# aehogan/lammps-induced-dipole-polarization-pair-style

Hardware: AMD Instinct MI355X
Metric: atom-steps/sec (higher is better)
Workload: dtype f64

## Files before the change

lammps-induced-dipole-polarization-pair-style_amd/csrc/polar_api.hip:

```cpp
#include "polar_handle.hpp"

namespace {
void upload_types(polar_handle *h, int ntypes, const double *const t[7]) {
  need_device(h);
  std::vector<double> pack;
  const double r_cmax = pack_lj_table(ntypes, t, pack);
  h->d_lj.ensure(pack.size());
  HIPCHECK(hipMemcpy(h->d_lj.p, pack.data(), pack.size() * sizeof(double), hipMemcpyHostToDevice));
  h->P.ntypes = ntypes;
  h->P.ljpack = h->d_lj.p;
  h->ntypes = ntypes;
  h->types_set = true;
  h->r_cmax = r_cmax;
  h->skin_valid = false;
}

void upload_coul(polar_handle *h, double g_ewald, double qqrd2e, const double *slj, const double *scoul, int nbits,
                 int mask, int shift, double tabinnersq, const double *const t[8]) {
  need_device(h);
  h->P.g_ewald = g_ewald; h->P.qqrd2e = qqrd2e;
  for (int k = 0; k < 4; k++) { h->P.special_lj[k] = slj[k]; h->P.special_coul[k] = scoul[k]; }
  h->P.ncoultablebits = nbits; h->P.ncoulmask = mask; h->P.ncoulshiftbits = shift; h->P.tabinnersq = tabinnersq;
  std::vector<double> pack;
  pack_coul_table(nbits, t, pack);
// ... 156 lines not shown
    return POLAR_OK;
  }
  return guarded(h, [&]() {
    HIPCHECK(hipSetDevice(device));
    h->device_set = true;
    h->stream.create();
    for (auto &e : h->ev) e.create();
    {
      int prio_lo = 0, prio_hi = 0;
      HIPCHECK(hipDeviceGetStreamPriorityRange(&prio_lo, &prio_hi));
      h->lj_stream.create(hipStreamNonBlocking, prio_lo);
    }
    h->ev_fork.create(); h->ev_join.create();
    h->ev_lj0.create(); h->ev_lj1.create();
    h->ev_dl0.create(hipEventDisableTiming); h->ev_dl1.create(hipEventDisableTiming);
    h->ev_mu_ready.create(hipEventDisableTiming);
    for (auto &e : h->ev_fchunk) e.create(hipEventDisableTiming);
    for (auto &e : h->ev_ks) e.create();
    h->dl_stream.create(hipStreamNonBlocking);
    if (getenv("POLAR_NO_OVERLAP")) h->overlap_lj = false;
    if (const char *e = getenv("POLAR_LJ_PERS")) h->lj_pers = atoi(e);
    if (const char *e = getenv("POLAR_LJ_SKIN")) h->lj_skin = atoi(e) != 0;
    if (const char *e = getenv("POLAR_NL_INERT")) h->nl_inert = atoi(e) != 0;
    if (const char *e = getenv("POLAR_LJ_PERS_THREADS")) h->lj_pers_threads = std::max(256, std::min(POLAR_LJ_PERS_THREADS, (atoi(e) / 64) * 64));
    { int ncu = 0; if (hipDeviceGetAttribute(&ncu, hipDeviceAttributeMultiprocessorCount, device) == hipSuccess) h->ncu = ncu; }
    h->h_scal.ensure(1);
    h->h_flags.ensure(16);
    h->h_ddtot.ensure(64 * 16);
    h->d_overflow.ensure(16); h->d_ddtot.ensure(64 * 16);
    h->d_scal.ensure(1);
    h->d_slots.ensure((size_t)POLAR_NSLOT * POLAR_SLOT_STRIDE);
    h->have_device = true;
    return POLAR_OK;
  });
}

int polar_destroy(polar_handle *h) {
  if (!h) return POLAR_OK;
  delete h;
  return POLAR_OK;
}

const char *polar_last_error(const polar_handle *h) { return h ? h->err.c_str() : "null handle"; }
const char *polar_last_warning(const polar_handle *h) { return h ? h->warn.c_str() : ""; }

int polar_pair_settings(polar_handle *h, int narg, const char *const *arg) {
// ... 711 lines not shown
```

lammps-induced-dipole-polarization-pair-style_amd/csrc/polar_common.hpp:

```cpp
#pragma once

#include <hip/hip_runtime.h>
#include <stdint.h>

#ifdef POLAR_LAB
#define POLAR_LAB_PARAM , int ablate
#define POLAR_LAB_PASS , ablate
#define POLAR_ABL(bit) (ablate & (bit))
#else
#define POLAR_LAB_PARAM
#define POLAR_LAB_PASS
#define POLAR_ABL(bit) 0
#endif

namespace polar {


struct __attribute__((aligned(64))) AtomRec {
  double x, mx;
  double y, my;
  double z, mz;
  double q, a;
};

// ... 222 lines not shown

struct RecQuad { double2 a, b, c, d; };
__device__ __forceinline__ RecQuad fetch_records(const AtomRec *__restrict__ rec, int j, double2 *stage, int lane) {
  const int q4 = lane >> 2;
  const char *base = reinterpret_cast<const char *>(rec);
  const unsigned piece = (unsigned)(lane & 3) * 16u, k = lane & 3;
  const unsigned j0 = __shfl(j, q4, 64), j1 = __shfl(j, 16 + q4, 64), j2 = __shfl(j, 32 + q4, 64), j3 = __shfl(j, 48 + q4, 64);
  const double2 p0 = *reinterpret_cast<const double2 *>(base + ((j0 << 6) + piece));
  const double2 p1 = *reinterpret_cast<const double2 *>(base + ((j1 << 6) + piece));
  const double2 p2 = *reinterpret_cast<const double2 *>(base + ((j2 << 6) + piece));
  const double2 p3 = *reinterpret_cast<const double2 *>(base + ((j3 << 6) + piece));
  stage[q4 * 5 + k] = p0; stage[(16 + q4) * 5 + k] = p1;
  stage[(32 + q4) * 5 + k] = p2; stage[(48 + q4) * 5 + k] = p3;
  __builtin_amdgcn_fence(__ATOMIC_RELEASE, "wavefront");
  __builtin_amdgcn_wave_barrier();
  __builtin_amdgcn_fence(__ATOMIC_ACQUIRE, "wavefront");
  RecQuad r;
  r.a = stage[lane * 5]; r.b = stage[lane * 5 + 1]; r.c = stage[lane * 5 + 2]; r.d = stage[lane * 5 + 3];
  __builtin_amdgcn_wave_barrier();
  return r;
}

struct XQ { double2 a, b; };
__device__ __forceinline__ XQ fetch_xq(const double4 *__restrict__ xq, int j, double2 *stage, int lane) {
  const int h2 = lane >> 1;
  const char *base = reinterpret_cast<const char *>(xq);
  const unsigned piece = (unsigned)(lane & 1) * 16u, k = lane & 1;
  const unsigned j0 = __shfl(j, h2, 64), j1 = __shfl(j, 32 + h2, 64);
  const double2 p0 = *reinterpret_cast<const double2 *>(base + ((j0 << 5) + piece));
  const double2 p1 = *reinterpret_cast<const double2 *>(base + ((j1 << 5) + piece));
  stage[h2 * 3 + k] = p0; stage[(32 + h2) * 3 + k] = p1;
  __builtin_amdgcn_fence(__ATOMIC_RELEASE, "wavefront");
  __builtin_amdgcn_wave_barrier();
  __builtin_amdgcn_fence(__ATOMIC_ACQUIRE, "wavefront");
  XQ r;
  r.a = stage[lane * 3]; r.b = stage[lane * 3 + 1];
  __builtin_amdgcn_wave_barrier();
  return r;
}

struct ExpCoef {
  double log2e, ln2hi, ln2lo;
  double c[14];
};
inline ExpCoef make_expcoef() {
  ExpCoef K;
  K.log2e = 1.4426950408889634074; K.ln2hi = 6.93147180369123816490e-01; K.ln2lo = 1.90821492927058770002e-10;
  const double c[14] = {1.0, 1.0, 0.5, 0.16666666666666666, 0.041666666666666664, 0.008333333333333333, 0.001388888888888889, 0.0001984126984126984, 2.48015873015873e-05, 2.7557319223985893e-06, 2.755731922398589e-07, 2.505210838544172e-08, 2.08767569878681e-09, 1.6059043836821613e-10};
  for (int k = 0; k < 14; k++) K.c[k] = c[k];
  return K;
}
__device__ __forceinline__ double exp_neg(double x, const ExpCoef &K) {
  x = fmax(x, -745.0);
  const double n = rint(x * K.log2e);
  double r = fma(-n, K.ln2hi, x);
  r = fma(-n, K.ln2lo, r);
  double p = K.c[13];
#pragma unroll
  for (int k = 12; k >= 0; k--) p = fma(p, r, K.c[k]);
  return ldexp(p, (int)n);
}
// ... 88 lines not shown
```

lammps-induced-dipole-polarization-pair-style_amd/csrc/polar_handle.hpp:

```cpp
#pragma once
#include <hip/hip_runtime.h>

#include <algorithm>
#include <initializer_list>
#include <utility>
#include <chrono>
#include <cmath>
#include <cstdio>
#include <cstdlib>
#include <exception>
#include <cstring>
#include <numeric>
#include <string>
#include <thread>
#include <mutex>
#include <condition_variable>
#include <functional>
#include <memory>
#include <stdexcept>
#include <unistd.h>
#include <vector>

#include "pair_host.hpp"
#include "polar_input.hpp"
// ... 60 lines not shown
  DBuf<double> d_ef_s, d_T6, d_Minv, d_gsN, d_gsAT, d_cb, d_gs_part, d_eatom, d_vatom, d_dd_r2, d_fpol;
  bool dense_gs = false;
  CellGrid grid{};
  long long ncell = 0;
  bool sorted = false;
  DBuf<long long> d_first, d_sym_first;
  DBuf<int> d_gs_cnt;
  DBuf<long long> d_scan_a, d_scan_b;
  DBuf<int> d_sym_cnt, d_sym_fill, d_sym_j;
  bool sym_valid = false;
  DBuf<long long> d_sym_cfirst;
  DBuf<int> d_sym_cend, d_lj_walk;
  DBuf<unsigned char> d_sym_cls;
  DBuf<double4> d_xq_snap;
  DBuf<unsigned long long> d_lj_drift;
  double r_cmax = 0.0;
  int lj_skin = 1;
  bool skin_valid = false;
  int skin_nall = 0;
  bool lj_ran = false;
  bool lj_sym_last = false, lj_walk_last = false; int lj_rows_last = 0;
  double lj_walked = 0.0, lj_entries = 0.0;
  int nl_inert = 1;
  bool force_ran = false, force_listed = false; int force_nrows = 0;
  double nl_entries = 0.0, force_rows = 0.0;
  DBuf<unsigned long long> d_inert_sums;
  DBuf<AtomRec> d_rec0, d_rec1;
  DBuf<Scal> d_scal;
  DBuf<double> d_slots;
  DBuf<int> d_cell_id, d_cell_cnt, d_cell_fill, d_nl_cnt, d_dd_cnt, d_nl_j, d_dd_j, d_dd_wrap;
  DBuf<long long> d_cell_first, d_nl_first, d_dd_first;
  DBuf<double2> d_dd_s;
  DBuf<int2> d_lpdesc;
  DBuf<double> d_lp_pend;
  DBuf<double> d_lp_part;
  int lp_npart = 0;
  DBuf<int> d_slot;
  std::vector<int> h_cl;
  DBuf<int> d_cl_orig, d_cl_cnt, d_cl_wrap, d_cl_tw;
  DBuf<int4> d_cl_s;
  long long cl_pitch = 0;
  int ncl = 0;
  double cluster_dist = 2.0;
  int cluster_max = 4;
  long long cl_slots = 0;
  DBuf<double4> d_xq, d_pos4, d_xq_s;
  long long nl_pairs = 0, dd_pairs = 0;
  long long nl_pitch = 0, dd_pitch = 0;
  DBuf<int> d_overflow;
  DBuf<unsigned long long> d_ddtot;
  PinBuf<int> h_flags;
  PinBuf<unsigned long long> h_ddtot;
  int inum = 0;
// ... 301 lines not shown
```

lammps-induced-dipole-polarization-pair-style_amd/csrc/polar_lists.hpp:

```cpp
#pragma once

#include "polar_common.hpp"
#include "polar_nl_dense.hpp"

namespace polar {

struct CellGrid {
  int trim;
  int nc[3];
  double lo[3], inv[3];
};

__device__ __forceinline__ int cell_of(const CellGrid &g, const Box &b, double x, double y, double z) {
  int c[3];
  double fr3[3];
  frac_coords(b, g.lo, x, y, z, fr3);
#pragma unroll
  for (int k = 0; k < 3; k++) {
    double fr = fr3[k];
    fr -= floor(fr);
    int ck = (int)(fr * g.nc[k]);
    c[k] = ck >= g.nc[k] ? g.nc[k] - 1 : ck;
  }
  return (c[2] * g.nc[1] + c[1]) * g.nc[0] + c[0];
// ... 446 lines not shown

__device__ __forceinline__ int prefix_count(unsigned long long m, int base) {
  return __builtin_amdgcn_mbcnt_hi((unsigned)(m >> 32), __builtin_amdgcn_mbcnt_lo((unsigned)m, base));
}
struct NlRunLanes {
  int s0v, k0v, s1v, k1v, endv;
  unsigned m1;
  __device__ __forceinline__ int s0(int sr) const { return __builtin_amdgcn_readlane(s0v, sr); }
  __device__ __forceinline__ int k0(int sr) const { return __builtin_amdgcn_readlane(k0v, sr); }
  __device__ __forceinline__ int s1(int sr) const { return __builtin_amdgcn_readlane(s1v, sr); }
  __device__ __forceinline__ int k1(int sr) const { return __builtin_amdgcn_readlane(k1v, sr); }
  __device__ __forceinline__ int end(int sr) const { return __builtin_amdgcn_readlane(endv, sr); }
  __device__ __forceinline__ bool two(int sr) const { return (m1 >> sr) & 1u; }
};
template <bool TRI, bool RECHECK, bool DENSE = true>
static __global__ __launch_bounds__(POLAR_BLOCK) void k_nl_build(const int *__restrict__ rows, int nrows,
                                                          const double4 *__restrict__ pos4, Box box, CellGrid g,
                                                          const long long *__restrict__ cell_first, double cutallsq,
                                                          double ddcutsq, long long nl_pitch, long long dd_pitch,
                                                          int *__restrict__ nl_cnt, int *__restrict__ dd_cnt,
                                                          int *__restrict__ nl_j, int *__restrict__ dd_j,
                                                          double *__restrict__ dd_r2, int pad_dd,
                                                          int dd_shift_qm, int dd_pad_index, int *__restrict__ dd_wrap,
                                                          const int *__restrict__ color_s, double colordistsq,
                                                          int *__restrict__ color_conflict,
                                                          const int *__restrict__ dd_slot,
                                                          int *__restrict__ overflow,
                                                          unsigned long long *__restrict__ dd_total) {
  const int dd_shift = dd_shift_qm & 255, dd_qm = dd_shift_qm >> 8;
  const int lane = threadIdx.x & 63;
  const int row = blockIdx.x * POLAR_ROWS_PER_BLOCK + (threadIdx.x >> 6);
  if (row >= nrows) return;
  const int i = __builtin_amdgcn_readfirstlane(rows ? rows[row] : row);
  const double4 ri = pos4[i];
  const int imol = __double2hiint(ri.w), ipol = __double2loint(ri.w) >= SITE_POLAR;
  const int icol = (RECHECK && color_s && ipol) ? color_s[i] : -2;
  bool clash = RECHECK && color_s && ipol && icol < 0;
  int cc[3];
  double uu[3], edge[3];
  {
    double fr3[3];
    frac_coords(box, g.lo, ri.x, ri.y, ri.z, fr3);
#pragma unroll
    for (int k = 0; k < 3; k++) {
      double fr = fr3[k];
      fr -= floor(fr);
      const double t = fr * g.nc[k];
      int ck = (int)t;
      ck = ck >= g.nc[k] ? g.nc[k] - 1 : ck;
      cc[k] = __builtin_amdgcn_readfirstlane(ck);
      uu[k] = wave_uniform(t - ck); edge[k] = wave_uniform(box.prd[k] / g.nc[k]);
    }
  }
  const int c0 = cc[0], c1 = cc[1], c2 = cc[2];
  const int slot_i = __builtin_amdgcn_readfirstlane(dd_slot ? dd_slot[i] : i);
  const long long nl0 = (long long)i * nl_pitch, dd0 = (long long)(slot_i >= 0 ? slot_i : 0) * dd_pitch;
  char *const nl_row = reinterpret_cast<char *>(nl_j + nl0), *const dd_row = reinterpret_cast<char *>(dd_j + dd0);
  char *const r2_row = reinterpret_cast<char *>(dd_r2 ? dd_r2 + dd0 : nullptr);
  const char *const pos_b = reinterpret_cast<const char *>(pos4);
  const int nl_cap = (int)nl_pitch, dd_cap = (int)dd_pitch;
  const unsigned long long dd_im = (ipol && slot_i >= 0) ? ~0ull : 0ull;
  Box pbox = box;
#pragma unroll
  for (int k = 0; k < 3; k++) { pbox.inv[k] = box.periodic[k] ? box.inv[k] : 0.0; pbox.periodic[k] = 1; }
  int ncount = 0, dcount = 0;
  unsigned long long wrap_m = 0ull;
  const int same_i = imol != 0 ? POLAR_NL_SAMEMOL : 0;
  const unsigned long long below = (lane == 0) ? 0ull : (~0ull >> (64 - lane));
  const int n0 = g.nc[0], n1 = g.nc[1], n2 = g.nc[2];
  const int zlo = n2 >= 5 ? c2 - 2 : 0, zcnt = n2 >= 5 ? 5 : n2;
  const int ylo = n1 >= 5 ? c1 - 2 : 0, ycnt = n1 >= 5 ? 5 : n1;
  const double reach = sqrt(cutallsq > ddcutsq ? cutallsq : ddcutsq) + 1e-6;
  const double reach2 = wave_uniform(reach * reach);
  const int nsr = zcnt * ycnt;
  int ra0 = 0, rb0 = 0, ra1 = 0, rb1 = 0;
  if (lane < nsr) {
    const int lz = (lane >= ycnt) + (lane >= 2 * ycnt) + (lane >= 3 * ycnt) + (lane >= 4 * ycnt);
    const int zz = zlo + lz, yy = ylo + (lane - lz * ycnt);
    int b2 = zz, b1 = yy;
    bool ok = true;
    if (b2 < 0 || b2 >= n2) { if (!box.periodic[2]) ok = false; b2 = b2 < 0 ? b2 + n2 : b2 - n2; }
    if (b1 < 0 || b1 >= n1) { if (!box.periodic[1]) ok = false; b1 = b1 < 0 ? b1 + n1 : b1 - n1; }
    double dzmin = 0.0, dymin = 0.0;
    if (n2 >= 5) { const int d = zz - c2; dzmin = d > 0 ? (d - uu[2]) * edge[2] : (d < 0 ? (uu[2] - (d + 1)) * edge[2] : 0.0); }
    if (n1 >= 5) { const int d = yy - c1; dymin = d > 0 ? (d - uu[1]) * edge[1] : (d < 0 ? (uu[1] - (d + 1)) * edge[1] : 0.0); }
    const double rem2 = reach2 - dzmin * dzmin - dymin * dymin;
    if (g.trim && rem2 < 0.0) ok = false;
    int xlo = n0 >= 5 ? c0 - 2 : 0, xhi = n0 >= 5 ? c0 + 2 : n0 - 1;
    if (ok && g.trim && n0 >= 5) {
// ... 3 lines not shown
      xlo = c0 + lo_off; xhi = c0 + hi_off;
    }
    if (ok) {
      const long long rowbase = ((long long)b2 * n1 + b1) * n0;
      const int xa = xlo < 0 ? 0 : xlo, xb = xhi >= n0 ? n0 - 1 : xhi;
      ra0 = (int)cell_first[rowbase + xa]; rb0 = (int)cell_first[rowbase + xb + 1];
      if (box.periodic[0]) {
        if (xlo < 0) { ra1 = (int)cell_first[rowbase + xlo + n0]; rb1 = (int)cell_first[rowbase + n0]; }
        else if (xhi >= n0) { ra1 = (int)cell_first[rowbase]; rb1 = (int)cell_first[rowbase + xhi - n0 + 1]; }
      }
    }
  }
  auto candidate = [&](const int p, const bool valid) {
    const int j = valid ? p : i;
    const double4 rj = *reinterpret_cast<const double4 *>(pos_b + ((unsigned)j << 5));
    double ex, ey, ez;
    const unsigned long long shifted = min_image_rint_m<TRI>(pbox, ri.x, ri.y, ri.z, rj.x, rj.y, rj.z, ex, ey, ez);
    const double rsq = ex * ex + ey * ey + ez * ez;
    const unsigned long long m_pair = __builtin_amdgcn_ballot_w64(j != i);
    const int jkind = __double2loint(rj.w);
    const unsigned long long m_nl = m_pair & __builtin_amdgcn_ballot_w64(rsq <= cutallsq) & __builtin_amdgcn_ballot_w64(jkind != SITE_INERT);
    const unsigned long long m_dd = m_pair & dd_im & __builtin_amdgcn_ballot_w64(jkind >= SITE_POLAR) & __builtin_amdgcn_ballot_w64(rsq < ddcutsq);
    wrap_m |= m_dd & shifted;
    const bool in_nl = (j != i) & (rsq <= cutallsq) & (jkind != SITE_INERT);
    const bool in_dd = (j != i) & (dd_im != 0ull) & (jkind >= SITE_POLAR) & (rsq < ddcutsq);
    if (RECHECK) { if (icol >= 0 && j != i && rsq < colordistsq && jkind >= SITE_POLAR && color_s[j] == icol) clash = true; }
    int jmol = __double2hiint(rj.w);
    asm("" : "+v"(jmol));
    const int same = imol == jmol ? same_i : 0;
    const int kn = prefix_count(m_nl, ncount), kd = prefix_count(m_dd, dcount);
    if (in_nl && kn < nl_cap) *reinterpret_cast<int *>(nl_row + ((unsigned)kn << 2)) = j | same;
    if (in_dd && kd < dd_cap) {
      *reinterpret_cast<int *>(dd_row + ((dd_shift ? lp_slot32((unsigned)kd, dd_qm) : (unsigned)kd) << 2)) = j << dd_shift;
      if (dd_r2) *reinterpret_cast<double *>(r2_row + ((unsigned)kd << 3)) = rsq;
    }
    ncount += __popcll(m_nl);
    dcount += __popcll(m_dd);
  };
  if (DENSE) {
    const int len = nl_run_len(ra0, rb0, ra1, rb1);
    int inc = len;
    inc += __builtin_amdgcn_update_dpp(0, inc, 0x111, 0xF, 0xF, true);
    inc += __builtin_amdgcn_update_dpp(0, inc, 0x112, 0xF, 0xF, true);
    inc += __builtin_amdgcn_update_dpp(0, inc, 0x114, 0xF, 0xF, true);
    inc += __builtin_amdgcn_update_dpp(0, inc, 0x118, 0xF, 0xF, true);
    const int row0 = __builtin_amdgcn_readlane(inc, 15);
// ... 8 lines not shown
      candidate(g + k, g < total);
    }
  } else {
    for (int sr = 0; sr < nsr; sr++) {
#pragma unroll
      for (int piece = 0; piece < 2; piece++) {
        const int a = __builtin_amdgcn_readlane(piece ? ra1 : ra0, sr), b = __builtin_amdgcn_readlane(piece ? rb1 : rb0, sr);
        for (int base = a; base < b; base += 64) candidate(base + lane, base + lane < b);
      }
    }
  }
  if (pad_dd) {
    const int have = dcount < dd_pitch ? dcount : (int)dd_pitch;
    const int padded = (have + 63) & ~63;
    for (int k = have + lane; k < padded; k += 64) {
      dd_j[dd0 + (dd_shift ? lp_slot(k, dd_qm) : (long long)k)] = (dd_pad_index >= 0 ? dd_pad_index : i) << dd_shift;
      if (dd_r2) dd_r2[dd0 + k] = 1e60;
    }
  }
  if (RECHECK && color_s && __ballot(clash) != 0ull && lane == 0) atomicOr(color_conflict, 1);
  if (lane == 0) {
    nl_cnt[i] = ncount; dd_cnt[i] = dcount;
    if (dd_wrap) dd_wrap[i] = wrap_m != 0ull;
    if (ncount > nl_pitch || dcount > dd_pitch) atomicMax(overflow, ncount > dcount ? ncount : dcount);
    if (dcount) atomicAdd(dd_total + (blockIdx.x & 63) * 16, (unsigned long long)(dcount < dd_pitch ? dcount : (int)dd_pitch));
  }
}

#ifdef POLAR_LAB
#include "lab/lists_paired_rows.hpp"
#endif

#ifdef POLAR_LAB
#include "lab/lists_cluster_rows.hpp"
#endif

struct LJGrid {
  int nc[3];
  double lo[3], inv[3];
};
__device__ __forceinline__ int lj_cell_of(const LJGrid &g, double x, double y, double z) {
  const double p[3] = {x, y, z};
  int c[3];
#pragma unroll
  for (int k = 0; k < 3; k++) {
    int ck = (int)floor((p[k] - g.lo[k]) * g.inv[k]);
// ... 230 lines not shown
```

lammps-induced-dipole-polarization-pair-style_amd/csrc/polar_rows.hpp:

```cpp
#pragma once

#include "polar_common.hpp"
#include "polar_force_pair.hpp"
#include "polar_skin.hpp"
#ifdef POLAR_LAB
#include "lab/force_pair_literal.hpp"
#define POLAR_LIT_PARAM , int literal
#define POLAR_LIT_PASS , literal
#else
#define POLAR_LIT_PARAM
#define POLAR_LIT_PASS
#endif

namespace polar {

static __global__ void k_pack(int n, const int *__restrict__ perm, const double *__restrict__ x, const double *__restrict__ q,
                       const double *__restrict__ alpha, const int *__restrict__ mol, const double *__restrict__ mu0,
                       AtomRec *__restrict__ r0, AtomRec *__restrict__ r1, int *__restrict__ mol_s,
                       double4 *__restrict__ pos4, double4 *__restrict__ xq_s, int wrap, Box box, double lo0, double lo1,
                       double lo2, int keep_inert) {
  int i = blockIdx.x * blockDim.x + threadIdx.x;
  if (i == n) {
    AtomRec d;
    d.x = n > 0 ? x[0] : 0.0; d.y = n > 0 ? x[1] : 0.0; d.z = n > 0 ? x[2] : 0.0;
// ... 444 lines not shown
    const double2 fdf = bin[1], ede = bin[2];
    ctab_lds[b] = make_double4(fdf.x, fdf.y, ede.x, ede.y);
  }
  __syncthreads();
  const int lane = threadIdx.x & 63, wv = threadIdx.x >> 6, nwv = blockDim.x >> 6;
  double ev = 0.0, ec = 0.0;
  for (int ii = blockIdx.x + gridDim.x * wv; ii < inum; ii += gridDim.x * nwv) {
    const int i = ilist ? ilist[ii] : ii;
    const int jnum = numneigh ? numneigh[i] : (int)(first[i + 1] - first[i]);
    if (jnum == 0) continue;
    double v[6] = {0, 0, 0, 0, 0, 0};
    ljcoul_row<EFLAG, VPAIR, TAB>(P, i, jnum, neigh + first[i], xq[i], xq, type, lj_lds, ctab_lds, lane, f, eatom, vatom, ev, ec, v);
    if (VPAIR) ljcoul_tally<false, true>(slots, ii, lane, vglobal, 0.0, 0.0, v);
  }
  const double none[6] = {0, 0, 0, 0, 0, 0};
  ljcoul_tally<EFLAG, false>(slots, blockIdx.x * nwv + wv, lane, 0, ev, ec, none);
}

template <bool ALLPAIRS, bool EW>
static __device__ __forceinline__ void static_field_body(const int *__restrict__ rows, int nrows, int nlocal,
                                                              const AtomRec *__restrict__ rec,
                                                              const int *__restrict__ mol, Box box,
                                                              RowList nl,
                                                              const int *__restrict__ nl_j, double cut_coulsq,
                                                              double e2s, double gamma, int use_previous,
                                                              double *__restrict__ ef, AtomRec *__restrict__ rec0,
                                                              AtomRec *__restrict__ rec1, const double4 *__restrict__ xq_s,
                                                              double g_ewald, const double *__restrict__ erec) {
  const int lane = threadIdx.x & 63;
  const int row = blockIdx.x * POLAR_ROWS_PER_BLOCK + (threadIdx.x >> 6);
  if (row >= nrows) return;
  const int i = rows ? rows[row] : row;
  const AtomRec ri = uniform_rec(rec[i]);
  const int mi = mol[i];
  const double f_shift = -1.0 / cut_coulsq;
  double ex = 0, ey = 0, ez = 0;
  long long beg = 0, end = nlocal;
  if (!ALLPAIRS) row_range(nl, i, beg, end);
  if (ALLPAIRS) {
    for (long long p = beg + lane; p < end; p += 64) {
      const int j = (int)p;
      if (j == i) continue;
      const AtomRec rj = rec[j];
      double dx, dy, dz;
      pair_del<ALLPAIRS>(box, ri.x, ri.y, ri.z, rj.x, rj.y, rj.z, dx, dy, dz);
      const double rsq = dx * dx + dy * dy + dz * dz;
      if (EW) {
        if (rsq <= cut_coulsq) {
          const double ef_temp = ewald_b1(rsq, g_ewald, (mi != mol[j]) || mi == 0) * rj.q;
          ex += ef_temp * dx; ey += ef_temp * dy; ez += ef_temp * dz;
        }
      } else if (rsq <= cut_coulsq && ((mi != mol[j]) || mi == 0)) {
        const double rinv = rsqrt(rsq);
        const double ef_temp = (rinv * rinv + f_shift) * rinv * rj.q;
        ex += ef_temp * dx; ey += ef_temp * dy; ez += ef_temp * dz;
      }
    }
  } else {
    __shared__ double2 s_stage[POLAR_ROWS_PER_BLOCK][64 * 5];
    double2 *stage = s_stage[threadIdx.x >> 6];
    for (long long base = beg; base < end; base += 64) {
      const long long p = base + lane;
      const bool valid = p < end;
      const int e = valid ? nl_j[p] : i;
      const int j = e & POLAR_NL_MASK;
      double xj, yj, zj, qj;
      if (xq_s) { const XQ t = fetch_xq(xq_s, j, stage, lane); xj = t.a.x; yj = t.a.y; zj = t.b.x; qj = t.b.y; }
      else { const RecQuad rj = fetch_records(rec, j, stage, lane); xj = rj.a.x; yj = rj.b.x; zj = rj.c.x; qj = rj.d.x; }
      double dx, dy, dz;
      pair_del<ALLPAIRS>(box, ri.x, ri.y, ri.z, xj, yj, zj, dx, dy, dz);
      const double rsq = dx * dx + dy * dy + dz * dz;
      if (EW) {
        if (valid && j != i && rsq <= cut_coulsq) {
          const double ef_temp = ewald_b1(rsq, g_ewald, !(e & POLAR_NL_SAMEMOL)) * qj;
          ex += ef_temp * dx; ey += ef_temp * dy; ez += ef_temp * dz;
        }
      } else if (valid && j != i && rsq <= cut_coulsq && !(e & POLAR_NL_SAMEMOL)) {
        const double rinv = rsqrt(rsq);
        const double ef_temp = (rinv * rinv + f_shift) * rinv * qj;
        ex += ef_temp * dx; ey += ef_temp * dy; ez += ef_temp * dz;
      }
    }
  }
  ex = wave_sum(ex); ey = wave_sum(ey); ez = wave_sum(ez);
  if (lane == 0) {
    ex *= e2s; ey *= e2s; ez *= e2s;
    if (EW) { ex += erec[3 * i]; ey += erec[3 * i + 1]; ez += erec[3 * i + 2]; }
    ef[3 * i] = ex; ef[3 * i + 1] = ey; ef[3 * i + 2] = ez;
    if (!use_previous) {
      const double a = ri.a;
      double mx = a * ex, my = a * ey, mz = a * ez;
      mx *= gamma; my *= gamma; mz *= gamma;
      rec0[i].mx = mx; rec0[i].my = my; rec0[i].mz = mz;
      rec1[i].mx = mx; rec1[i].my = my; rec1[i].mz = mz;
    }
  }
}

template <bool ALLPAIRS>
static __global__ __launch_bounds__(POLAR_BLOCK) void k_static_field(const int *__restrict__ rows, int nrows, int nlocal,
                                                              const AtomRec *__restrict__ rec,
                                                              const int *__restrict__ mol, Box box,
                                                              RowList nl,
                                                              const int *__restrict__ nl_j, double cut_coulsq,
                                                              double e2s, double gamma, int use_previous,
                                                              double *__restrict__ ef, AtomRec *__restrict__ rec0,
                                                              AtomRec *__restrict__ rec1, const double4 *__restrict__ xq_s) {
  static_field_body<ALLPAIRS, false>(rows, nrows, nlocal, rec, mol, box, nl, nl_j, cut_coulsq, e2s, gamma, use_previous, ef, rec0, rec1,
                                     xq_s, 0.0, nullptr);
}
template <bool ALLPAIRS>
static __global__ __launch_bounds__(POLAR_BLOCK) void k_ew_static_field(const int *__restrict__ rows, int nrows, int nlocal,
                                                                 const AtomRec *__restrict__ rec,
                                                                 const int *__restrict__ mol, Box box,
                                                                 RowList nl,
                                                                 const int *__restrict__ nl_j, double cut_coulsq,
                                                                 double e2s, double gamma, int use_previous,
                                                                 double *__restrict__ ef, AtomRec *__restrict__ rec0,
                                                                 AtomRec *__restrict__ rec1, const double4 *__restrict__ xq_s,
                                                                 double g_ewald, const double *__restrict__ erec) {
  static_field_body<ALLPAIRS, true>(rows, nrows, nlocal, rec, mol, box, nl, nl_j, cut_coulsq, e2s, gamma, use_previous, ef, rec0, rec1,
                                    xq_s, g_ewald, erec);
}

struct PairMath {
  const ExpCoef &K;
  double g_ewald;
  __device__ __forceinline__ double rsqrt(double x) const { return rsqrt_pos3(x); }
  __device__ __forceinline__ double exp_neg(double x) const { return exp_neg_fast<12>(x, K); }
  __device__ __forceinline__ void ewald_b12(double rsq, bool kept, double &b1, double &b2) const { polar::ewald_b12(rsq, g_ewald, kept, b1, b2); }
};

template <bool ALLPAIRS, int DAMP, bool EFLAG, bool VPAIR, bool EW>
static __device__ __forceinline__ void polar_force_body(const int *__restrict__ rows, int nrows, const int *__restrict__ perm,
                                                             int nlocal, const Scal *scal_in,
                                                             const AtomRec *__restrict__ recA,
                                                             const AtomRec *__restrict__ recB,
                                                             const int *__restrict__ mol, Box box,
                                                             RowList nl,
                                                             const int *__restrict__ nl_j, double cut_coulsq,
                                                             double ddcutsq, double pd, double e2s,
                                                             double *__restrict__ f, double *__restrict__ slots,
                                                             double *__restrict__ vatom, int vglobal, ExpCoef K,
                                                             double *__restrict__ dbg6, double g_ewald, int skip_inert POLAR_LIT_PARAM) {
// ... 136 lines not shown
```

lammps-induced-dipole-polarization-pair-style_amd/csrc/polar_step.hip:

```cpp
#include "polar_handle.hpp"

void launch_scan(long long n, const int *in, long long *out, DBuf<long long> &tot, hipStream_t s) {
  const int nb = (int)std::max<long long>(1, (n + POLAR_SCAN_ITEMS - 1) / POLAR_SCAN_ITEMS);
  tot.ensure((size_t)nb + 1);
  k_scan_block<<<nb, 1024, 0, s>>>(n, in, out, tot.p);
  if (nb > 1) {
    k_scan_totals<<<1, 1024, 0, s>>>(nb, tot.p, out + n);
    k_scan_add<<<nblk(n - POLAR_SCAN_ITEMS, 256), 256, 0, s>>>(n, out, tot.p);
  }
}

void build_cells(polar_handle *h) {
  const polar_settings &st = h->ph.st;
  const int n = h->nlocal;
  const double cutall = std::max(st.cut_coul, st.dd_cutoff);
  double width[3];
  box_widths(h->box, width);
  CellGrid &g = h->grid;
  if (!list_grid(width, h->box.periodic, cutall, g.nc))
    throw InputError("dd_cutoff mode needs box lengths >= 2*max(cut_coul,dd_cutoff); use exact mode (dd_cutoff 0)");
  g.trim = 1;
#ifdef POLAR_LAB
  if (const char *e = getenv("POLAR_NL_TRIM")) g.trim = atoi(e);
#endif
// ... 61 lines not shown
  } else {
    k_slot_from_rows<<<nblk(own_n(h), 256), 256, 0, s>>>(own_n(h), own_rows(h), h->d_slot.p);
    h->slots_by_color = false;
  }
}

void build_lists(polar_handle *h) {
  const polar_settings &st = h->ph.st;
  const int n = h->nlocal;
  const double cutall = std::max(st.cut_coul, st.dd_cutoff);
  hipStream_t s = h->stream;
  const CellGrid &g = h->grid;
  if (h->nl_pitch == 0 && getenv("POLAR_INIT_PITCH")) h->nl_pitch = h->dd_pitch = pitch_forced(atoi(getenv("POLAR_INIT_PITCH")));
  if (h->nl_pitch == 0) {
    const double vol = occupied_volume(n, h->hx.data(), g.lo, h->box.prd, cutall);
    h->dens = n / vol;
    double mean = n / vol * 4.18879020478639 * cutall * cutall * cutall;
    h->nl_pitch = h->dd_pitch = pitch_first(mean, 1.5);
  }
  if (h->sweep_kernel == 2) h->dd_pitch = ((h->dd_pitch + 255) / 256) * 256;
  if ((h->sweep_kernel == 2 || h->sweep_kernel == 3) && ((long long)n + 1) * (long long)sizeof(AtomRec) >= (1ll << 31))
    throw InputError("more than 2^25 atoms on one handle: the 32-bit record offsets of the sweep's index stream would wrap (shard the system)");
  h->d_nl_cnt.ensure(n + 1); h->d_dd_cnt.ensure(n + 1);
  h->d_nl_j.ensure((size_t)n * h->nl_pitch + 64);
  if (h->sweep_kernel < 3) h->d_dd_j.ensure((size_t)n * h->dd_pitch + 1024);
  else h->d_dd_j.ensure(64);
  const int mode = h->stream_mode = stream_mode(h->cache_r2, h->sweep_kernel, h->dd_pairs, own_n(h), h->dd_pitch);
  const bool r2c = mode == 1;
  if (mode == 1) h->d_dd_r2.ensure((size_t)n * h->dd_pitch + 64);
  else if (mode == 0) h->d_dd_s.ensure((size_t)n * h->dd_pitch + 64);
  double *r2p = r2c ? h->d_dd_r2.p : nullptr;
  double2 *sp = mode == 0 ? h->d_dd_s.p : nullptr;
  bool fuse = mode != 0 && mode != 4;
#ifdef POLAR_LAB
  if (getenv("POLAR_NO_FUSE_R2")) fuse = false;
#endif
  const double cutallsq = cutall * cutall, ddsq = mode == 4 ? -1.0 : st.dd_cutoff * st.dd_cutoff;
  const int nr = own_n(h);
  const int *rows = own_rows(h);
  zero_many(s, {{h->d_nl_cnt.p, (size_t)(n + 1) * sizeof(int)}, {h->d_dd_cnt.p, (size_t)(n + 1) * sizeof(int)},
                {h->d_overflow.p, 16 * sizeof(int)}, {h->d_ddtot.p, 64 * 16 * sizeof(unsigned long long)}});
  const bool lp = mode == 3;
  if (lp) h->d_dd_wrap.ensure(n + 1);
  const bool recheck = h->colors_valid && h->colors_recheck && h->sweep_kernel < 3 && (int)h->h_color.size() == n;
  if (h->colors_recheck && !recheck) { h->colors_valid = false; h->colors_recheck = false; }
  if (recheck) {
    h->d_color_s.ensure(n + 1);
    k_color_map<<<nblk(n, 256), 256, 0, s>>>(n, h->d_perm.p, h->d_color_orig.p, h->d_color_s.p);
  }
  if (((long long)n + 1) * (long long)sizeof(double4) >= (1ll << 32))
    throw InputError("more than 2^27 atoms on one handle: the 32-bit position offsets of the list build would wrap (shard the system)");
#define NLB3(TRI, RC, DENSE)                                                                                                  \
  k_nl_build<TRI, RC, DENSE><<<nblk(nr, POLAR_ROWS_PER_BLOCK), POLAR_BLOCK, 0, s>>>(                                          \
      rows, nr, h->d_pos4.p, h->box, g, h->d_cell_first.p, cutallsq, ddsq, h->nl_pitch, h->dd_pitch, h->d_nl_cnt.p,            \
      h->d_dd_cnt.p, h->d_nl_j.p, h->d_dd_j.p, fuse ? r2p : nullptr, fuse ? 1 : 0, lp ? (6 | (h->lp_quad_major << 8)) : 0,    \
      lp ? n : -1, lp ? h->d_dd_wrap.p : nullptr, recheck ? h->d_color_s.p : nullptr, h->color_keep * h->color_keep,           \
      h->d_overflow.p + 8, lp ? h->d_slot.p : nullptr, h->d_overflow.p, h->d_ddtot.p)
#ifdef POLAR_LAB
#define NLB(TRI, RC) do { if (h->nl_dense) NLB3(TRI, RC, true); else NLB3(TRI, RC, false); } while (0)
  h->nl_dense_used = h->nl_dense ? 1.0 : 0.0;
#else
#define NLB(TRI, RC) NLB3(TRI, RC, true)
#endif
  if (h->box.triclinic) { if (recheck) NLB(true, true); else NLB(true, false); }
  else                  { if (recheck) NLB(false, true); else NLB(false, false); }
#undef NLB
#undef NLB3
  const RowList ddl{h->d_dd_cnt.p, h->dd_pitch};
  if (fuse || mode == 4) {
  }
#ifdef POLAR_LAB
  else if (st.damping_type == POLAR_DAMP_EXPONENTIAL)
    k_dd_scalars<0><<<nblk(nr, POLAR_ROWS_PER_BLOCK), POLAR_BLOCK, 0, s>>>(rows, nr, h->d_rec0.p, h->box, ddl, h->d_dd_j.p, st.polar_damp, sp, r2p);
  else
    k_dd_scalars<1><<<nblk(nr, POLAR_ROWS_PER_BLOCK), POLAR_BLOCK, 0, s>>>(rows, nr, h->d_rec0.p, h->box, ddl, h->d_dd_j.p, st.polar_damp, sp, r2p);
#endif
  HIPCHECK(hipMemcpyAsync(h->h_flags.p, h->d_overflow.p, sizeof(int), hipMemcpyDeviceToHost, s));
  HIPCHECK(hipMemcpyAsync(h->h_ddtot.p, h->d_ddtot.p, 64 * 16 * sizeof(unsigned long long), hipMemcpyDeviceToHost, s));
}
// ... 662 lines not shown
  if (!ap) {
    if (h->colors_valid && h->sweep_kernel < 3) map_color_rows(h);
    if (h->sweep_kernel == 2) compute_slots(h);
    build_lists(h);
    if (h->colors_valid && h->sweep_kernel == 3) build_cluster_lists(h);
    if (h->sweep_kernel == 4) build_tiles(h);
  }
  HIPCHECK(hipEventRecord(h->ev[1], s));

  if (st.polar_gs_ranked && (ap || (!h->colors_valid && h->sweep_kernel != 4)) && !ranked_done) {
    if (ap) { launch_rank<true>(h, 1); launch_rank<true>(h, 2); }
    else    { launch_rank<false>(h, 1); launch_rank<false>(h, 2); }
  }
  HIPCHECK(hipEventRecord(h->ev[2], s));

  HIPCHECK(hipEventRecord(h->ev[3], s));

  {
    dim3 grid(nblk(own_n(h), POLAR_ROWS_PER_BLOCK)), block(POLAR_BLOCK);
    const double ccs = st.cut_coul * st.cut_coul, e2s = std::sqrt(h->P.qqrd2e);
    if (ewald_on(h)) {
      ewald_field(h);
      const double g = h->P.g_ewald;
      if (ap) k_ew_static_field<true><<<grid, block, 0, s>>>(nullptr, n, n, h->d_rec0.p, h->d_mol_s.p, h->box, RowList{nullptr, 0}, nullptr, ccs, e2s, st.polar_gamma, st.use_previous, h->d_ef_s.p, h->d_rec0.p, h->d_rec1.p, nullptr, g, h->d_ew_erec.p);
      else    k_ew_static_field<false><<<grid, block, 0, s>>>(own_rows(h), own_n(h), n, h->d_rec0.p, h->d_mol_s.p, h->box, RowList{h->d_nl_cnt.p, h->nl_pitch}, h->d_nl_j.p, ccs, e2s, st.polar_gamma, st.use_previous, h->d_ef_s.p, h->d_rec0.p, h->d_rec1.p, h->static_xq ? h->d_xq_s.p : nullptr, g, h->d_ew_erec.p);
    } else if (ap) k_static_field<true><<<grid, block, 0, s>>>(nullptr, n, n, h->d_rec0.p, h->d_mol_s.p, h->box, RowList{nullptr, 0}, nullptr, ccs, e2s, st.polar_gamma, st.use_previous, h->d_ef_s.p, h->d_rec0.p, h->d_rec1.p, nullptr);
    else    k_static_field<false><<<grid, block, 0, s>>>(own_rows(h), own_n(h), n, h->d_rec0.p, h->d_mol_s.p, h->box, RowList{h->d_nl_cnt.p, h->nl_pitch}, h->d_nl_j.p, ccs, e2s, st.polar_gamma, st.use_previous, h->d_ef_s.p, h->d_rec0.p, h->d_rec1.p, h->static_xq ? h->d_xq_s.p : nullptr);
  }
#ifdef POLAR_LAB
  if (!ap && h->sweep_kernel == 4 && !st.zodid)
    k_srec_pack<<<nblk(n, 256), 256, 0, s>>>(n, h->d_rec0.p, h->d_srec0.p, h->d_srec1.p);
#endif
  HIPCHECK(hipEventRecord(h->ev[4], s));
  if (lj_late) launch_lj();
}

int phase_finish(polar_handle *h, polar_result *out) {
  const polar_settings &st = h->ph.st;
  const int n = h->nlocal, nall = h->nlocal + h->nghost;
  const bool ap = !(st.dd_cutoff > 0.0);
  const bool expd = st.damping_type == POLAR_DAMP_EXPONENTIAL;
  const int eflag = h->step_eflag, vmode = h->step_vflag % 4;
  hipStream_t s = h->stream;
#ifdef POLAR_LAB
  if (!ap && h->sweep_kernel == 4 && !st.zodid)
    k_srec_unpack<<<nblk(n, 256), 256, 0, s>>>(n, h->d_scal.p, h->d_srec0.p, h->d_srec1.p, h->d_rec0.p, h->d_rec1.p);
#endif
  k_fallback<<<nblk(n, 256), 256, 0, s>>>(n, h->d_scal.p, h->d_rec0.p, h->d_rec1.p, h->d_ef_s.p);
  HIPCHECK(hipEventRecord(h->ev[5], s));
  k_unpack<<<nblk(n, 256), 256, 0, s>>>(n, h->sorted ? h->d_perm.p : nullptr, h->d_scal.p, h->d_rec0.p, h->d_rec1.p, h->d_ef_s.p, h->d_mu.p, h->d_ef.p);
// ... 169 lines not shown
```

Before: 16.74 million.

## Prefetch neighbor indices and positions in static field, skip minimum-image for unwrapped rows

```diff
diff --git a/lammps-induced-dipole-polarization-pair-style_amd/csrc/polar_api.hip b/lammps-induced-dipole-polarization-pair-style_amd/csrc/polar_api.hip
--- a/lammps-induced-dipole-polarization-pair-style_amd/csrc/polar_api.hip
+++ b/lammps-induced-dipole-polarization-pair-style_amd/csrc/polar_api.hip
@@ -202,6 +202,7 @@
     if (const char *e = getenv("POLAR_LJ_PERS")) h->lj_pers = atoi(e);
     if (const char *e = getenv("POLAR_LJ_SKIN")) h->lj_skin = atoi(e) != 0;
     if (const char *e = getenv("POLAR_NL_INERT")) h->nl_inert = atoi(e) != 0;
+    if (const char *e = getenv("POLAR_NL_WRAP")) h->nl_wrap = atoi(e) != 0;
     if (const char *e = getenv("POLAR_LJ_PERS_THREADS")) h->lj_pers_threads = std::max(256, std::min(POLAR_LJ_PERS_THREADS, (atoi(e) / 64) * 64));
     { int ncu = 0; if (hipDeviceGetAttribute(&ncu, hipDeviceAttributeMultiprocessorCount, device) == hipSuccess) h->ncu = ncu; }
     h->h_scal.ensure(1);
diff --git a/lammps-induced-dipole-polarization-pair-style_amd/csrc/polar_common.hpp b/lammps-induced-dipole-polarization-pair-style_amd/csrc/polar_common.hpp
--- a/lammps-induced-dipole-polarization-pair-style_amd/csrc/polar_common.hpp
+++ b/lammps-induced-dipole-polarization-pair-style_amd/csrc/polar_common.hpp
@@ -268,14 +268,19 @@
 }
 
 struct XQ { double2 a, b; };
-__device__ __forceinline__ XQ fetch_xq(const double4 *__restrict__ xq, int j, double2 *stage, int lane) {
+__device__ __forceinline__ XQ fetch_xq_issue(const double4 *__restrict__ xq, int j, int lane) {
   const int h2 = lane >> 1;
   const char *base = reinterpret_cast<const char *>(xq);
-  const unsigned piece = (unsigned)(lane & 1) * 16u, k = lane & 1;
+  const unsigned piece = (unsigned)(lane & 1) * 16u;
   const unsigned j0 = __shfl(j, h2, 64), j1 = __shfl(j, 32 + h2, 64);
-  const double2 p0 = *reinterpret_cast<const double2 *>(base + ((j0 << 5) + piece));
-  const double2 p1 = *reinterpret_cast<const double2 *>(base + ((j1 << 5) + piece));
-  stage[h2 * 3 + k] = p0; stage[(32 + h2) * 3 + k] = p1;
+  XQ p;
+  p.a = *reinterpret_cast<const double2 *>(base + ((j0 << 5) + piece));
+  p.b = *reinterpret_cast<const double2 *>(base + ((j1 << 5) + piece));
+  return p;
+}
+__device__ __forceinline__ XQ fetch_xq_land(const XQ &p, double2 *stage, int lane) {
+  const int h2 = lane >> 1, k = lane & 1;
+  stage[h2 * 3 + k] = p.a; stage[(32 + h2) * 3 + k] = p.b;
   __builtin_amdgcn_fence(__ATOMIC_RELEASE, "wavefront");
   __builtin_amdgcn_wave_barrier();
   __builtin_amdgcn_fence(__ATOMIC_ACQUIRE, "wavefront");
@@ -283,6 +288,9 @@
   r.a = stage[lane * 3]; r.b = stage[lane * 3 + 1];
   __builtin_amdgcn_wave_barrier();
   return r;
+}
+__device__ __forceinline__ XQ fetch_xq(const double4 *__restrict__ xq, int j, double2 *stage, int lane) {
+  return fetch_xq_land(fetch_xq_issue(xq, j, lane), stage, lane);
 }
 
 struct ExpCoef {
diff --git a/lammps-induced-dipole-polarization-pair-style_amd/csrc/polar_handle.hpp b/lammps-induced-dipole-polarization-pair-style_amd/csrc/polar_handle.hpp
--- a/lammps-induced-dipole-polarization-pair-style_amd/csrc/polar_handle.hpp
+++ b/lammps-induced-dipole-polarization-pair-style_amd/csrc/polar_handle.hpp
@@ -106,13 +106,14 @@
   bool lj_sym_last = false, lj_walk_last = false; int lj_rows_last = 0;
   double lj_walked = 0.0, lj_entries = 0.0;
   int nl_inert = 1;
+  int nl_wrap = 1;
   bool force_ran = false, force_listed = false; int force_nrows = 0;
   double nl_entries = 0.0, force_rows = 0.0;
   DBuf<unsigned long long> d_inert_sums;
   DBuf<AtomRec> d_rec0, d_rec1;
   DBuf<Scal> d_scal;
   DBuf<double> d_slots;
-  DBuf<int> d_cell_id, d_cell_cnt, d_cell_fill, d_nl_cnt, d_dd_cnt, d_nl_j, d_dd_j, d_dd_wrap;
+  DBuf<int> d_cell_id, d_cell_cnt, d_cell_fill, d_nl_cnt, d_dd_cnt, d_nl_j, d_dd_j, d_dd_wrap, d_nl_wrap;
   DBuf<long long> d_cell_first, d_nl_first, d_dd_first;
   DBuf<double2> d_dd_s;
   DBuf<int2> d_lpdesc;
diff --git a/lammps-induced-dipole-polarization-pair-style_amd/csrc/polar_lists.hpp b/lammps-induced-dipole-polarization-pair-style_amd/csrc/polar_lists.hpp
--- a/lammps-induced-dipole-polarization-pair-style_amd/csrc/polar_lists.hpp
+++ b/lammps-induced-dipole-polarization-pair-style_amd/csrc/polar_lists.hpp
@@ -492,6 +492,7 @@
                                                           int *__restrict__ nl_j, int *__restrict__ dd_j,
                                                           double *__restrict__ dd_r2, int pad_dd,
                                                           int dd_shift_qm, int dd_pad_index, int *__restrict__ dd_wrap,
+                                                          int *__restrict__ nl_wrap,
                                                           const int *__restrict__ color_s, double colordistsq,
                                                           int *__restrict__ color_conflict,
                                                           const int *__restrict__ dd_slot,
@@ -535,6 +536,7 @@
   for (int k = 0; k < 3; k++) { pbox.inv[k] = box.periodic[k] ? box.inv[k] : 0.0; pbox.periodic[k] = 1; }
   int ncount = 0, dcount = 0;
   unsigned long long wrap_m = 0ull;
+  unsigned long long nlwrap_m = 0ull;
   const int same_i = imol != 0 ? POLAR_NL_SAMEMOL : 0;
   const unsigned long long below = (lane == 0) ? 0ull : (~0ull >> (64 - lane));
   const int n0 = g.nc[0], n1 = g.nc[1], n2 = g.nc[2];
@@ -584,6 +586,7 @@
     const unsigned long long m_nl = m_pair & __builtin_amdgcn_ballot_w64(rsq <= cutallsq) & __builtin_amdgcn_ballot_w64(jkind != SITE_INERT);
     const unsigned long long m_dd = m_pair & dd_im & __builtin_amdgcn_ballot_w64(jkind >= SITE_POLAR) & __builtin_amdgcn_ballot_w64(rsq < ddcutsq);
     wrap_m |= m_dd & shifted;
+    nlwrap_m |= m_nl & shifted;
     const bool in_nl = (j != i) & (rsq <= cutallsq) & (jkind != SITE_INERT);
     const bool in_dd = (j != i) & (dd_im != 0ull) & (jkind >= SITE_POLAR) & (rsq < ddcutsq);
     if (RECHECK) { if (icol >= 0 && j != i && rsq < colordistsq && jkind >= SITE_POLAR && color_s[j] == icol) clash = true; }
@@ -638,6 +641,7 @@
   if (lane == 0) {
     nl_cnt[i] = ncount; dd_cnt[i] = dcount;
     if (dd_wrap) dd_wrap[i] = wrap_m != 0ull;
+    if (nl_wrap) nl_wrap[i] = TRI || nlwrap_m != 0ull;
     if (ncount > nl_pitch || dcount > dd_pitch) atomicMax(overflow, ncount > dcount ? ncount : dcount);
     if (dcount) atomicAdd(dd_total + (blockIdx.x & 63) * 16, (unsigned long long)(dcount < dd_pitch ? dcount : (int)dd_pitch));
   }
diff --git a/lammps-induced-dipole-polarization-pair-style_amd/csrc/polar_rows.hpp b/lammps-induced-dipole-polarization-pair-style_amd/csrc/polar_rows.hpp
--- a/lammps-induced-dipole-polarization-pair-style_amd/csrc/polar_rows.hpp
+++ b/lammps-induced-dipole-polarization-pair-style_amd/csrc/polar_rows.hpp
@@ -490,7 +490,8 @@
                                                               const AtomRec *__restrict__ rec,
                                                               const int *__restrict__ mol, Box box,
                                                               RowList nl,
-                                                              const int *__restrict__ nl_j, double cut_coulsq,
+                                                              const int *__restrict__ nl_j,
+                                                              const int *__restrict__ nl_wrap, double cut_coulsq,
                                                               double e2s, double gamma, int use_previous,
                                                               double *__restrict__ ef, AtomRec *__restrict__ rec0,
                                                               AtomRec *__restrict__ rec1, const double4 *__restrict__ xq_s,
@@ -499,12 +500,23 @@
   const int row = blockIdx.x * POLAR_ROWS_PER_BLOCK + (threadIdx.x >> 6);
   if (row >= nrows) return;
   const int i = rows ? rows[row] : row;
+  long long beg = 0, end = nlocal;
+  int e_n1 = i, e_n2 = i, cnt = 0, wrapped = 1;
+  if (!ALLPAIRS) {
+    beg = (long long)i * nl.pitch;
+    e_n1 = nl_j[beg + lane]; e_n2 = nl_j[beg + lane + 64];
+    cnt = nl.cnt[i];
+    if (nl_wrap) wrapped = __builtin_amdgcn_readfirstlane(nl_wrap[i]);
+  }
   const AtomRec ri = uniform_rec(rec[i]);
   const int mi = mol[i];
   const double f_shift = -1.0 / cut_coulsq;
   double ex = 0, ey = 0, ez = 0;
-  long long beg = 0, end = nlocal;
-  if (!ALLPAIRS) row_range(nl, i, beg, end);
+  if (!ALLPAIRS) {
+    end = beg + (cnt < nl.pitch ? cnt : nl.pitch);
+    if (!(beg + lane < end)) e_n1 = i;
+    if (!(beg + lane + 64 < end)) e_n2 = i;
+  }
   if (ALLPAIRS) {
     for (long long p = beg + lane; p < end; p += 64) {
       const int j = (int)p;
@@ -527,16 +539,22 @@
   } else {
     __shared__ double2 s_stage[POLAR_ROWS_PER_BLOCK][64 * 5];
     double2 *stage = s_stage[threadIdx.x >> 6];
+    XQ xq_n{};
+    if (xq_s) xq_n = fetch_xq_issue(xq_s, e_n1 & POLAR_NL_MASK, lane);
     for (long long base = beg; base < end; base += 64) {
       const long long p = base + lane;
       const bool valid = p < end;
-      const int e = valid ? nl_j[p] : i;
+      const int e = e_n1;
       const int j = e & POLAR_NL_MASK;
       double xj, yj, zj, qj;
-      if (xq_s) { const XQ t = fetch_xq(xq_s, j, stage, lane); xj = t.a.x; yj = t.a.y; zj = t.b.x; qj = t.b.y; }
+      if (xq_s) { const XQ t = fetch_xq_land(xq_n, stage, lane); xj = t.a.x; yj = t.a.y; zj = t.b.x; qj = t.b.y; }
       else { const RecQuad rj = fetch_records(rec, j, stage, lane); xj = rj.a.x; yj = rj.b.x; zj = rj.c.x; qj = rj.d.x; }
+      e_n1 = e_n2;
+      if (xq_s && base + 64 < end) xq_n = fetch_xq_issue(xq_s, e_n1 & POLAR_NL_MASK, lane);
+      e_n2 = p + 128 < end ? nl_j[p + 128] : i;
       double dx, dy, dz;
-      pair_del<ALLPAIRS>(box, ri.x, ri.y, ri.z, xj, yj, zj, dx, dy, dz);
+      if (wrapped) pair_del<ALLPAIRS>(box, ri.x, ri.y, ri.z, xj, yj, zj, dx, dy, dz);
+      else { dx = ri.x - xj; dy = ri.y - yj; dz = ri.z - zj; }
       const double rsq = dx * dx + dy * dy + dz * dz;
       if (EW) {
         if (valid && j != i && rsq <= cut_coulsq) {
@@ -570,11 +588,12 @@
                                                               const AtomRec *__restrict__ rec,
                                                               const int *__restrict__ mol, Box box,
                                                               RowList nl,
-                                                              const int *__restrict__ nl_j, double cut_coulsq,
+                                                              const int *__restrict__ nl_j,
+                                                              const int *__restrict__ nl_wrap, double cut_coulsq,
                                                               double e2s, double gamma, int use_previous,
                                                               double *__restrict__ ef, AtomRec *__restrict__ rec0,
                                                               AtomRec *__restrict__ rec1, const double4 *__restrict__ xq_s) {
-  static_field_body<ALLPAIRS, false>(rows, nrows, nlocal, rec, mol, box, nl, nl_j, cut_coulsq, e2s, gamma, use_previous, ef, rec0, rec1,
+  static_field_body<ALLPAIRS, false>(rows, nrows, nlocal, rec, mol, box, nl, nl_j, nl_wrap, cut_coulsq, e2s, gamma, use_previous, ef, rec0, rec1,
                                      xq_s, 0.0, nullptr);
 }
 template <bool ALLPAIRS>
@@ -582,12 +601,13 @@
                                                                  const AtomRec *__restrict__ rec,
                                                                  const int *__restrict__ mol, Box box,
                                                                  RowList nl,
-                                                                 const int *__restrict__ nl_j, double cut_coulsq,
+                                                                 const int *__restrict__ nl_j,
+                                                                 const int *__restrict__ nl_wrap, double cut_coulsq,
                                                                  double e2s, double gamma, int use_previous,
                                                                  double *__restrict__ ef, AtomRec *__restrict__ rec0,
                                                                  AtomRec *__restrict__ rec1, const double4 *__restrict__ xq_s,
                                                                  double g_ewald, const double *__restrict__ erec) {
-  static_field_body<ALLPAIRS, true>(rows, nrows, nlocal, rec, mol, box, nl, nl_j, cut_coulsq, e2s, gamma, use_previous, ef, rec0, rec1,
+  static_field_body<ALLPAIRS, true>(rows, nrows, nlocal, rec, mol, box, nl, nl_j, nl_wrap, cut_coulsq, e2s, gamma, use_previous, ef, rec0, rec1,
                                     xq_s, g_ewald, erec);
 }
 
diff --git a/lammps-induced-dipole-polarization-pair-style_amd/csrc/polar_step.hip b/lammps-induced-dipole-polarization-pair-style_amd/csrc/polar_step.hip
--- a/lammps-induced-dipole-polarization-pair-style_amd/csrc/polar_step.hip
+++ b/lammps-induced-dipole-polarization-pair-style_amd/csrc/polar_step.hip
@@ -107,7 +107,8 @@
   if ((h->sweep_kernel == 2 || h->sweep_kernel == 3) && ((long long)n + 1) * (long long)sizeof(AtomRec) >= (1ll << 31))
     throw InputError("more than 2^25 atoms on one handle: the 32-bit record offsets of the sweep's index stream would wrap (shard the system)");
   h->d_nl_cnt.ensure(n + 1); h->d_dd_cnt.ensure(n + 1);
-  h->d_nl_j.ensure((size_t)n * h->nl_pitch + 64);
+  h->d_nl_j.ensure((size_t)n * h->nl_pitch + 128);
+  h->d_nl_wrap.ensure(n + 1);
   if (h->sweep_kernel < 3) h->d_dd_j.ensure((size_t)n * h->dd_pitch + 1024);
   else h->d_dd_j.ensure(64);
   const int mode = h->stream_mode = stream_mode(h->cache_r2, h->sweep_kernel, h->dd_pairs, own_n(h), h->dd_pitch);
@@ -139,7 +140,7 @@
   k_nl_build<TRI, RC, DENSE><<<nblk(nr, POLAR_ROWS_PER_BLOCK), POLAR_BLOCK, 0, s>>>(                                          \
       rows, nr, h->d_pos4.p, h->box, g, h->d_cell_first.p, cutallsq, ddsq, h->nl_pitch, h->dd_pitch, h->d_nl_cnt.p,            \
       h->d_dd_cnt.p, h->d_nl_j.p, h->d_dd_j.p, fuse ? r2p : nullptr, fuse ? 1 : 0, lp ? (6 | (h->lp_quad_major << 8)) : 0,    \
-      lp ? n : -1, lp ? h->d_dd_wrap.p : nullptr, recheck ? h->d_color_s.p : nullptr, h->color_keep * h->color_keep,           \
+      lp ? n : -1, lp ? h->d_dd_wrap.p : nullptr, h->d_nl_wrap.p, recheck ? h->d_color_s.p : nullptr, h->color_keep * h->color_keep,           \
       h->d_overflow.p + 8, lp ? h->d_slot.p : nullptr, h->d_overflow.p, h->d_ddtot.p)
 #ifdef POLAR_LAB
 #define NLB(TRI, RC) do { if (h->nl_dense) NLB3(TRI, RC, true); else NLB3(TRI, RC, false); } while (0)
@@ -848,10 +849,10 @@
     if (ewald_on(h)) {
       ewald_field(h);
       const double g = h->P.g_ewald;
-      if (ap) k_ew_static_field<true><<<grid, block, 0, s>>>(nullptr, n, n, h->d_rec0.p, h->d_mol_s.p, h->box, RowList{nullptr, 0}, nullptr, ccs, e2s, st.polar_gamma, st.use_previous, h->d_ef_s.p, h->d_rec0.p, h->d_rec1.p, nullptr, g, h->d_ew_erec.p);
-      else    k_ew_static_field<false><<<grid, block, 0, s>>>(own_rows(h), own_n(h), n, h->d_rec0.p, h->d_mol_s.p, h->box, RowList{h->d_nl_cnt.p, h->nl_pitch}, h->d_nl_j.p, ccs, e2s, st.polar_gamma, st.use_previous, h->d_ef_s.p, h->d_rec0.p, h->d_rec1.p, h->static_xq ? h->d_xq_s.p : nullptr, g, h->d_ew_erec.p);
-    } else if (ap) k_static_field<true><<<grid, block, 0, s>>>(nullptr, n, n, h->d_rec0.p, h->d_mol_s.p, h->box, RowList{nullptr, 0}, nullptr, ccs, e2s, st.polar_gamma, st.use_previous, h->d_ef_s.p, h->d_rec0.p, h->d_rec1.p, nullptr);
-    else    k_static_field<false><<<grid, block, 0, s>>>(own_rows(h), own_n(h), n, h->d_rec0.p, h->d_mol_s.p, h->box, RowList{h->d_nl_cnt.p, h->nl_pitch}, h->d_nl_j.p, ccs, e2s, st.polar_gamma, st.use_previous, h->d_ef_s.p, h->d_rec0.p, h->d_rec1.p, h->static_xq ? h->d_xq_s.p : nullptr);
+      if (ap) k_ew_static_field<true><<<grid, block, 0, s>>>(nullptr, n, n, h->d_rec0.p, h->d_mol_s.p, h->box, RowList{nullptr, 0}, nullptr, nullptr, ccs, e2s, st.polar_gamma, st.use_previous, h->d_ef_s.p, h->d_rec0.p, h->d_rec1.p, nullptr, g, h->d_ew_erec.p);
+      else    k_ew_static_field<false><<<grid, block, 0, s>>>(own_rows(h), own_n(h), n, h->d_rec0.p, h->d_mol_s.p, h->box, RowList{h->d_nl_cnt.p, h->nl_pitch}, h->d_nl_j.p, h->nl_wrap ? h->d_nl_wrap.p : nullptr, ccs, e2s, st.polar_gamma, st.use_previous, h->d_ef_s.p, h->d_rec0.p, h->d_rec1.p, h->static_xq ? h->d_xq_s.p : nullptr, g, h->d_ew_erec.p);
+    } else if (ap) k_static_field<true><<<grid, block, 0, s>>>(nullptr, n, n, h->d_rec0.p, h->d_mol_s.p, h->box, RowList{nullptr, 0}, nullptr, nullptr, ccs, e2s, st.polar_gamma, st.use_previous, h->d_ef_s.p, h->d_rec0.p, h->d_rec1.p, nullptr);
+    else    k_static_field<false><<<grid, block, 0, s>>>(own_rows(h), own_n(h), n, h->d_rec0.p, h->d_mol_s.p, h->box, RowList{h->d_nl_cnt.p, h->nl_pitch}, h->d_nl_j.p, h->nl_wrap ? h->d_nl_wrap.p : nullptr, ccs, e2s, st.polar_gamma, st.use_previous, h->d_ef_s.p, h->d_rec0.p, h->d_rec1.p, h->static_xq ? h->d_xq_s.p : nullptr);
   }
 #ifdef POLAR_LAB
   if (!ap && h->sweep_kernel == 4 && !st.zodid)
```

Measured after the change: 16.79 million, median of 6. About the same (+0.3%).
